# hbell99/DirectVoxGO

Measured on AMD Instinct MI355X. Metric: train rays/sec (8192-ray batch, 160^3 grid), higher is better.
Workload: dtype f32

## Files before the change

directvoxgo_amd/csrc/shade.hip:

```cpp
#include "common.h"
#include "x3.h"

#include <type_traits>


static int g_shade_experiment = 0;
static int g_shade_variant = 67;
extern "C" int dvgo_shade_wgrad_x3(const float* G1, const float* gz, const uint64_t* masks, const float* W3, const float* H1,
                                   const float* H2, const float* feat, int C, const float* emb, int E, const int64_t* ray_id,
                                   int64_t M, const int64_t* m_dev, int width, int diffuse, int n_parts, float* part, int form_b,
                                   void* stream);
extern "C" int dvgo_shade_bwd_x3(const float* g_rgb, const float* rgb, const uint64_t* masks, int64_t M, const int64_t* m_dev,
                                 const float* W1, const float* W2, const float* W3, int width, int d_in, int C, int diffuse,
                                 float* g_feat, float* G1, float* gz, void* scratch, int prebuilt, void* stream);

extern "C" int dvgo_shade_fwd_x3(const float* feat, int C, const float* emb, int E, const int64_t* ray_id, int64_t M, const int64_t* m_dev,
                                 const float* W1, const float* b1, const float* W2, const float* b2, const float* W3,
                                 const float* b3, int width, int d_in, int diffuse, float* rgb, float* H1, float* H2,
                                 uint64_t* masks, void* scratch, void* scratch_bwd, int experiment, void* stream);

#define SHADE_THREADS 768
#define SHADE_WAVES (SHADE_THREADS / 64)
#define SHADE_BWD_THREADS 1024
#define SHADE_BWD_WAVES (SHADE_BWD_THREADS / 64)
// ... 724 lines not shown
    if (j < 8) pb[2 * WIDTH + 8 * w + j] = (w == 0 && j < 3) ? sgz[j] : 0.0f;
    if (T == 2 && j >= 16) pb[2 * WIDTH + 16 * w + j] = 0.0f;
  }
#endif
}
typedef float dvgo_f32x2 __attribute__((ext_vector_type(2)));
template <int O0, int O1> __device__ __forceinline__ dvgo_f32x2 lds_f32_pair_st64(unsigned a) {
  dvgo_f32x2 v; asm volatile("ds_read2st64_b32 %0, %1 offset0:%2 offset1:%3" : "=v"(v) : "v"(a), "n"(O0), "n"(O1)); return v;
}
template <int O0, int O1> __device__ __forceinline__ dvgo_f32x2 lds_f32_pair(unsigned a) {
  dvgo_f32x2 v; asm volatile("ds_read2_b32 %0, %1 offset0:%2 offset1:%3" : "=v"(v) : "v"(a), "n"(O0), "n"(O1)); return v;
}
template <int OFF> __device__ __forceinline__ u32x4 lds_u32x4(unsigned a) {
  u32x4 v; asm volatile("ds_read_b128 %0, %1 offset:%2" : "=v"(v) : "v"(a), "n"(OFF)); return v;
}
template <int OFF> __device__ __forceinline__ void lds_store_u32x4(unsigned a, u32x4 v) {
  asm volatile("ds_write_b128 %0, %1 offset:%2" :: "v"(a), "v"(v), "n"(OFF) : "memory");
}

template <int WIDTH>
struct ShadeWgradRingX3 : ShadeWgradRing<WIDTH> {
  u32x4 fb[WIDTH / 32 + 2][3][64];
};

template <int WIDTH>
__global__ void __launch_bounds__(2 * WIDTH, 2)
shade_wgrad_ring_x3_kernel(const float* __restrict__ G1, const float* __restrict__ gz, const unsigned int* __restrict__ masks,
                           const float* __restrict__ W3, const float* __restrict__ H1, const float* __restrict__ H2,
                           const float* __restrict__ feat, int C, int c_view0, int n_view, const float* __restrict__ emb, int E,
                           const int64_t* __restrict__ ray_id, int64_t M_cap, const int64_t* __restrict__ m_dev,
// ... 231 lines not shown
#pragma unroll
  for (int c = 0; c < 3; ++c) {
    const float v = vW3[c] + __shfl_xor(vW3[c], 32);
    if (h == 0) pW3[c * WIDTH + 32 * w + j] = v;
    sgz[c] += __shfl_xor(sgz[c], 32);
  }
  sb1 += __shfl_xor(sb1, 32); sb2 += __shfl_xor(sb2, 32);
  if (h == 0) {
    pb[32 * w + j] = sb1;
    pb[WIDTH + 32 * w + j] = sb2;
    if (j < 8) pb[2 * WIDTH + 8 * w + j] = (w == 0 && j < 3) ? sgz[j] : 0.0f;
    if (T == 2 && j >= 16) pb[2 * WIDTH + 16 * w + j] = 0.0f;
  }
#endif
}
#undef DVGO_OOB

#define SHADE_REDUCE_SLICES 16
__global__ void __launch_bounds__(256)
shade_wgrad_reduce_kernel(const float* __restrict__ part, int n_parts, int n, int W, int d_in, float* __restrict__ out) {
  const int i = blockIdx.x * blockDim.x + threadIdx.x;
  if (i >= n) return;
  int o;
  const int nW2 = W * W, nW1 = W * 64, nW3 = 32 * W;
  if (i < nW2) o = i;
  else if (i < nW2 + nW1) {
    const int r = (i - nW2) >> 6, c = (i - nW2) & 63;
    o = c < d_in ? nW2 + r * d_in + c : -1;
  } else if (i < nW2 + nW1 + nW3) {
    const int e = i - nW2 - nW1;
// ... 18 lines not shown
    a3 += part[(int64_t)(p + 3) * n + i];
  }
  for (; p < p1; ++p) a0 += part[(int64_t)p * n + i];
  if (p1 > p0) atomicAdd(out + o, (a0 + a1) + (a2 + a3));
}

extern "C" {

int dvgo_shade_fwd(const float* feat, int C, const float* emb, int E, const int64_t* ray_id, int64_t M, const int64_t* m_dev,
                   const float* W1, const float* b1, const float* W2, const float* b2, const float* W3,
                   const float* b3, int width, int d_in, int diffuse, float* rgb, float* H1, float* H2,
                   uint64_t* masks, void* scratch, void* scratch_bwd, void* stream) {
  if (M < 0 || C <= 0 || E < 0) return DVGO_EINVAL;
  if (M == 0) return 0;
  if (!feat || !emb || !ray_id || !W1 || !b1 || !W2 || !b2 || !W3 || !b3 || !rgb) return DVGO_EINVAL;
  if ((H1 == nullptr) != (H2 == nullptr) || (H1 == nullptr) != (masks == nullptr)) return DVGO_EINVAL;
  const int c_view0 = diffuse ? 3 : 0;
  const int n_view = C - c_view0;
  if (n_view < 0 || d_in != n_view + E) return DVGO_EINVAL;
  if ((width != 128 && width != 64) || d_in > 40) return DVGO_ERANGE;
  if ((g_shade_variant & 1) && scratch != nullptr)
    return dvgo_shade_fwd_x3(feat, C, emb, E, ray_id, M, m_dev, W1, b1, W2, b2, W3, b3, width, d_in, diffuse, rgb, H1, H2, masks,
                             scratch, (g_shade_variant & 2) ? scratch_bwd : nullptr, g_shade_experiment, stream);
  hipStream_t s = (hipStream_t)stream;
  const int64_t n_tiles = (M + 31) / 32;
  const int64_t cap = width == 128 ? 256 : 512;
  int blocks = (int)((n_tiles + SHADE_WAVES - 1) / SHADE_WAVES < cap ? (n_tiles + SHADE_WAVES - 1) / SHADE_WAVES : cap);
#define DVGO_SHADE(W, S1, DIFF)                                                                           \
  shade_fwd_kernel<W, S1, DIFF><<<blocks, SHADE_THREADS, 0, s>>>(feat, C, c_view0, n_view, emb, E, ray_id, M, m_dev, W1, b1, W2, \
                                                          b2, W3, b3, d_in, rgb, H1, H2, (unsigned long long*)masks, g_shade_experiment)
  if (width == 128) {
    if (d_in <= 36) { if (diffuse) DVGO_SHADE(128, 18, true); else DVGO_SHADE(128, 18, false); }
    else            { if (diffuse) DVGO_SHADE(128, 20, true); else DVGO_SHADE(128, 20, false); }
  } else {
    if (d_in <= 12) { if (diffuse) DVGO_SHADE(64, 6, true); else DVGO_SHADE(64, 6, false); }
    else            { if (diffuse) DVGO_SHADE(64, 20, true); else DVGO_SHADE(64, 20, false); }
// ... 20 lines not shown
    return dvgo_shade_bwd_x3(g_rgb, rgb, masks, M, m_dev, W1, W2, W3, width, d_in, C, diffuse, g_feat, G1, gz, scratch, prebuilt, stream);
  hipStream_t s = (hipStream_t)stream;
  const int64_t n_tiles = (M + 31) / 32;
  const int64_t cap = width == 128 ? 256 : 512;
  int blocks = (int)((n_tiles + SHADE_BWD_WAVES - 1) / SHADE_BWD_WAVES < cap ? (n_tiles + SHADE_BWD_WAVES - 1) / SHADE_BWD_WAVES : cap);
#define DVGO_SHADE_BWD(W, DIFF)                                                                                                       \
  shade_bwd_kernel<W, DIFF><<<blocks, SHADE_BWD_THREADS, 0, s>>>(g_rgb, rgb, (const unsigned long long*)masks, M, m_dev, W1, W2, W3, d_in, C, c_view0, \
                                                            n_view, g_feat, G1, gz, g_shade_experiment)
  if (width == 128) { if (diffuse) DVGO_SHADE_BWD(128, true); else DVGO_SHADE_BWD(128, false); }
  else              { if (diffuse) DVGO_SHADE_BWD(64, true); else DVGO_SHADE_BWD(64, false); }
#undef DVGO_SHADE_BWD
  DVGO_LAUNCH_CHECK();
  return 0;
}

int dvgo_shade_wgrad(const float* G1, const float* gz, const uint64_t* masks, const float* W3, const float* H1,
                     const float* H2, const float* feat, int C, const float* emb, int E, const int64_t* ray_id, int64_t M,
                     const int64_t* m_dev, int width, int diffuse, int n_parts, float* part, float* total, void* stream) {
  if (M < 0 || n_parts <= 0 || C <= 0 || E < 0) return DVGO_EINVAL;
  if (!G1 || !gz || !masks || !W3 || !H1 || !H2 || !feat || !emb || !ray_id || !part || !total) return DVGO_EINVAL;
  const int c_view0 = diffuse ? 3 : 0;
  const int n_view = C - c_view0;
  if ((width != 128 && width != 64) || n_view < 0 || n_view + E > 40) return DVGO_ERANGE;
  bool ring = false;
  if (g_shade_variant & (4 | 32)) {
    const int form_b = (g_shade_variant & 32) ? 2 : (g_shade_variant & 16) ? 1 : 0;
    if (!form_b && n_parts > 256) n_parts = 256;
    const int rc = dvgo_shade_wgrad_x3(G1, gz, masks, W3, H1, H2, feat, C, emb, E, ray_id, M, m_dev, width, diffuse, n_parts, part,
                                       form_b, stream);
    if (rc != 0) return rc;
  } else if (!(g_shade_variant & 8) && n_view <= 16 && E <= 32 && (n_view + E <= 32 || (n_view % 4 == 0 && n_view >= 8)) &&
             M * width * 4 < ((int64_t)1 << 31) && M * C * 4 < ((int64_t)1 << 31)) {
    if (n_parts > 512) n_parts = 512;
    ring = true;
// ... 32 lines not shown
```

directvoxgo_amd/csrc/shade_x3.hip:

```cpp
#include "common.h"
#include "x3.h"

#ifndef X3_THREADS
#define X3_THREADS 512
#endif
#define X3_WAVES (X3_THREADS / 64)
#ifndef X3_BWD_THREADS
#define X3_BWD_THREADS 512
#endif
#define X3_BWD_WAVES (X3_BWD_THREADS / 64)
#define X3_STAGE_ROWS 16
#define X3_STAGE_STRIDE 36

__device__ __forceinline__ int x3_acc_feature(int t, int r, int h) { return 32 * t + (r & 3) + 8 * (r >> 2) + 4 * h; }

__device__ __forceinline__ void x3_split1(float v, unsigned short& s0, unsigned short& s1, unsigned short& s2) {
  const unsigned int h = x3_pack(v, 0.f) & 0xffffu;
  const float r = v - __uint_as_float(h << 16);
  const unsigned int m = x3_pack(r, 0.f) & 0xffffu;
  const float q = r - __uint_as_float(m << 16);
  s0 = (unsigned short)h; s1 = (unsigned short)m; s2 = (unsigned short)(x3_pack(q, 0.f) & 0xffffu);
}

template <int WIDTH, int KS1>
// ... 83 lines not shown
}

template <int WIDTH, int KS1, bool DIFFUSE>
__global__ void __launch_bounds__(X3_THREADS)
shade_fwd_x3_kernel(const float* __restrict__ feat, int C, int c_view0, int n_view, const float* __restrict__ emb, int E,
                    const int64_t* __restrict__ ray_id, int64_t M_cap, const int64_t* __restrict__ m_dev,
                    const void* __restrict__ image, float* __restrict__ rgb,
                    float* __restrict__ H1, float* __restrict__ H2, unsigned long long* __restrict__ masks, int experiment) {
  const int64_t M = m_dev ? (*m_dev < M_cap ? *m_dev : M_cap) : M_cap;
  constexpr int T = WIDTH / 32;
  __shared__ __attribute__((aligned(16))) X3Lds<WIDTH, KS1> L;
  x3_copy_image<X3Img<WIDTH, KS1>>(&L, image);
  __syncthreads();
  const int lane = threadIdx.x & 63, h = lane >> 5;
  float* stage = L.stage[threadIdx.x >> 6];
  const bool train = H1 != nullptr;
  const int64_t n_tiles = (M + 31) / 32;
  const int64_t gw = (int64_t)blockIdx.x * (blockDim.x >> 6) + (threadIdx.x >> 6);
  const int64_t nw = (int64_t)gridDim.x * (blockDim.x >> 6);
  const int d_in = n_view + E;
  const int64_t last = M > 0 ? M - 1 : 0;
  auto row_of = [&](int64_t tile) { const int64_t r = tile * 32 + (lane & 31); return r < M ? r : last; };
  float xin[KS1][8];
  auto load_inputs = [&](int64_t tile, int64_t rid) {
    const float* fr = feat + row_of(tile) * C + c_view0;
    const float* er = emb + rid * E - n_view;
#pragma unroll
    for (int s = 0; s < KS1; ++s)
#pragma unroll
      for (int j = 0; j < 8; ++j) {
        const int k = 16 * s + 8 * h + j;
// ... 22 lines not shown
#pragma unroll
    for (int t = 0; t < T; ++t) {
      f32x16 acc;
#pragma unroll
      for (int r = 0; r < 16; ++r) acc[r] = L.b1p[h][t * 16 + r];
#pragma unroll
      for (int s = 0; s < KS1; ++s)
        x3_mfma6(acc, L.w1s[t][s][0][lane], L.w1s[t][s][1][lane], L.w1s[t][s][2][lane], x3[s][0], x3[s][1], x3[s][2]);
#pragma unroll
      for (int r = 0; r < 16; ++r) acc[r] = dvgo_relu(acc[r]);
      if (train) {
        unsigned int bits = 0u;
#pragma unroll
        for (int r = 0; r < 16; ++r) bits |= dvgo_relu_bit(acc[r]) << r;
        mask1 |= (unsigned long long)bits << (16 * t);
        if (!(experiment & 512)) x3_store_tile(stage, acc, H1 + tile * 32 * WIDTH + 32 * t, WIDTH, lane, rows_valid);
      }
#pragma unroll
      for (int s2 = 0; s2 < 2; ++s2) {
        float v[8];
#pragma unroll
        for (int j = 0; j < 8; ++j) v[j] = acc[8 * s2 + j];
        x3_split8(v, h3[2 * t + s2][0], h3[2 * t + s2][1], h3[2 * t + s2][2]);
      }
      __builtin_amdgcn_sched_barrier(0);
    }
    float p[3] = {0.0f, 0.0f, 0.0f};
    unsigned long long mask2 = 0ull;
#pragma unroll 1
    for (int t2 = 0; t2 < T; ++t2) {
      f32x16 acc2;
// ... 908 lines not shown
extern "C" {

int64_t dvgo_shade_scratch_bytes(int width) {
  if (width == 128) return (int64_t)sizeof(X3Img<128, 3>) > (int64_t)sizeof(X3BwdImg<128>) ? sizeof(X3Img<128, 3>) : sizeof(X3BwdImg<128>);
  if (width == 64) return (int64_t)sizeof(X3Img<64, 3>) > (int64_t)sizeof(X3BwdImg<64>) ? sizeof(X3Img<64, 3>) : sizeof(X3BwdImg<64>);
  return 0;
}

int dvgo_shade_fwd_x3(const float* feat, int C, const float* emb, int E, const int64_t* ray_id, int64_t M, const int64_t* m_dev,
                      const float* W1, const float* b1, const float* W2, const float* b2, const float* W3,
                      const float* b3, int width, int d_in, int diffuse, float* rgb, float* H1, float* H2,
                      uint64_t* masks, void* scratch, void* scratch_bwd, int experiment, void* stream) {
  if (M < 0 || C <= 0 || E < 0) return DVGO_EINVAL;
  if (M == 0) return 0;
  if (!feat || !emb || !ray_id || !W1 || !b1 || !W2 || !b2 || !W3 || !b3 || !rgb || !scratch) return DVGO_EINVAL;
  if ((H1 == nullptr) != (H2 == nullptr) || (H1 == nullptr) != (masks == nullptr)) return DVGO_EINVAL;
  const int c_view0 = diffuse ? 3 : 0;
  const int n_view = C - c_view0;
  if (n_view < 0 || d_in != n_view + E) return DVGO_EINVAL;
  if ((width != 128 && width != 64) || d_in > 48) return DVGO_ERANGE;
  hipStream_t s = (hipStream_t)stream;
  const int64_t n_tiles = (M + 31) / 32;
  const int64_t cap = 256;
  const int blocks = (int)((n_tiles + X3_WAVES - 1) / X3_WAVES < cap ? (n_tiles + X3_WAVES - 1) / X3_WAVES : cap);
#define DVGO_SHADE_X3(W, KS, DIFF)                                                                                       \
  do {                                                                                                                   \
    x3_prep_fwd_kernel<W, KS><<<scratch_bwd ? 64 : 32, 256, 0, s>>>((X3Img<W, KS>*)scratch, (X3BwdImg<W>*)scratch_bwd, W1, b1, W2, b2, W3, b3, d_in); \
    shade_fwd_x3_kernel<W, KS, DIFF><<<blocks, X3_THREADS, 0, s>>>(feat, C, c_view0, n_view, emb, E, ray_id, M, m_dev, scratch, rgb, \
                                                                    H1, H2, (unsigned long long*)masks, experiment);     \
  } while (0)
  if (width == 128) {
// ... 71 lines not shown
```

directvoxgo_amd/shade.py:

```python

import torch
import torch.nn as nn

from . import _lib as L
from ._lib import _i64, _int, ptr, stream_of

N_PARTS = 512


class defer_wgrad:
    _active = None
    _streams = {}

    def __init__(self, side_stream=True):
        self.side_stream = side_stream

    def __enter__(self):
        self.pending = []
        defer_wgrad._active = self
        return self

    def __exit__(self, *exc):
        defer_wgrad._active = None
        return False
# ... 64 lines not shown
        defer_wgrad._active.submit(params, wgrad, device)
    else:
        grads[k:k + 6] = wgrad()
    return tuple(grads)


class _Shade(torch.autograd.Function):
    @staticmethod
    def forward(ctx, feat, emb, ray_id, W1, b1, W2, b2, W3, b3, diffuse, train, m_dev):
        M, C = feat.shape
        E = emb.shape[1]
        width, d_in = W1.shape
        feat, emb = feat.contiguous(), emb.contiguous()
        train = bool(train) and any(ctx.needs_input_grad)
        rgb = torch.empty((M, 3), dtype=torch.float32, device=feat.device)
        H1 = torch.empty((M, width), dtype=torch.float32, device=feat.device) if train else None
        H2 = torch.empty((M, width), dtype=torch.float32, device=feat.device) if train else None
        masks = torch.empty((M, 4), dtype=torch.int64, device=feat.device) if train else None
        scratch = _scratch(width, feat.device)
        scratch_bwd = _scratch(width, feat.device) if (train and (L.lib().dvgo_shade_variant(-1) & 2)) else None
        with L.device_of(feat):
            L.call('dvgo_shade_fwd', ptr(feat), _int(C), ptr(emb), _int(E), ptr(ray_id), _i64(M), ptr(m_dev), ptr(W1.contiguous()),
                   ptr(b1.contiguous()), ptr(W2.contiguous()), ptr(b2.contiguous()), ptr(W3.contiguous()),
                   ptr(b3.contiguous()), _int(width), _int(d_in), _int(1 if diffuse else 0), ptr(rgb), ptr(H1), ptr(H2),
                   ptr(masks), ptr(scratch), ptr(scratch_bwd), stream_of(feat))
        ctx.scratch_bwd = scratch_bwd if (train and (L.lib().dvgo_shade_variant(-1) & 1)) else None
        if train:
            ctx.save_for_backward(feat, emb, ray_id, W1, W2, W3, rgb, H1, H2, masks)
            ctx.diffuse = diffuse
            ctx.m_dev = m_dev
            ctx.params = (W1, b1, W2, b2, W3, b3)
            ctx.w_versions = (W1._version, W2._version, W3._version)
        return rgb

    @staticmethod
    @torch.autograd.function.once_differentiable
    def backward(ctx, g_rgb):
        feat, emb, ray_id, W1, W2, W3, rgb, H1, H2, masks = ctx.saved_tensors
        diffuse, m_dev = ctx.diffuse, ctx.m_dev
        M, C = feat.shape
        width, d_in = W1.shape
        g_feat = torch.empty_like(feat)
        G1 = torch.empty_like(H1)
        gz = torch.empty_like(rgb)
        prebuilt = ctx.scratch_bwd is not None and W1._version == ctx.w_versions[0] and W2._version == ctx.w_versions[1] \
            and W3._version == ctx.w_versions[2]
        scratch = ctx.scratch_bwd if prebuilt else _scratch(width, feat.device)
        ctx.scratch_bwd = None
        with L.device_of(feat):
            L.call('dvgo_shade_bwd', ptr(g_rgb.contiguous()), ptr(rgb), ptr(masks), _i64(M), ptr(m_dev), ptr(W1.contiguous()),
                   ptr(W2.contiguous()), ptr(W3.contiguous()), _int(width), _int(d_in), _int(C), _int(1 if diffuse else 0),
                   ptr(g_feat), ptr(G1), ptr(gz), ptr(scratch), _int(1 if prebuilt else 0), stream_of(feat))

        def wgrad():
            n_parts = max(1, min(N_PARTS, (M + 255) // 256))
            psize = width * width + width * 64 + 32 * width + 3 * width
            part = torch.empty((n_parts, psize), dtype=torch.float32, device=feat.device)
            tsize = width * width + width * d_in + 5 * width + 3
            tot = torch.empty(tsize, dtype=torch.float32, device=feat.device)
            with L.device_of(feat):
                L.call('dvgo_shade_wgrad', ptr(G1), ptr(gz), ptr(masks), ptr(W3.contiguous()), ptr(H1), ptr(H2), ptr(feat), _int(C), ptr(emb),
                       _int(emb.shape[1]), ptr(ray_id), _i64(M), ptr(m_dev), _int(width), _int(1 if diffuse else 0), _int(n_parts),
                       ptr(part), ptr(tot), stream_of(feat))
            return _unpack_record(tot, width, d_in)

        return _weight_grads(ctx.params, wgrad, feat.device, 3, 12, g_feat if ctx.needs_input_grad[0] else None)


def shade(rgbnet, feat, emb, ray_id, diffuse, m_dev=None):
    layers = head_layers(rgbnet)
    if layers is None or not feat.is_cuda:
        return None
    l1, l2, l3 = layers
    c0 = 3 if diffuse else 0
    if l1.in_features != feat.shape[1] - c0 + emb.shape[1]:
# ... 92 lines not shown
```

include/dvgo_hip.h:

```cpp
#ifndef DVGO_HIP_H
#define DVGO_HIP_H

#include <stdint.h>

#ifdef __cplusplus
extern "C" {
#endif

#define DVGO_EINVAL (-1)
#define DVGO_ERANGE (-2)

#define DVGO_ABI_VERSION 11
int dvgo_abi_version(void);

#define DVGO_TUNE_FEAT_BWD    0
#define DVGO_TUNE_DENSITY_BWD 1
#define DVGO_TUNE_DENSITY_FWD 2
#define DVGO_TUNE_GATHER      3
#define DVGO_TUNE_EXPERIMENT  4
#define DVGO_TUNE_COUNT       8
int dvgo_set_tuning(int key, int value);

int dvgo_infer_t_minmax(const float* rays_o, const float* rays_d,
                        const float* xyz_min, const float* xyz_max,
// ... 176 lines not shown
                   void* stream);

int64_t dvgo_shade_scratch_bytes(int width);
int dvgo_shade_variant(int flags);

int dvgo_shade_bwd(const float* g_rgb, const float* rgb, const uint64_t* masks, int64_t M, const int64_t* m_dev,
                   const float* W1, const float* W2, const float* W3, int width, int d_in, int C, int diffuse,
                   float* g_feat, float* G1, float* gz, void* scratch,
                   int prebuilt ,
                   void* stream);

int dvgo_shade_wgrad(const float* G1, const float* gz, const uint64_t* masks, const float* W3,
                     const float* H1, const float* H2, const float* feat, int C, const float* emb, int E, const int64_t* ray_id, int64_t M,
                     const int64_t* m_dev, int width, int diffuse, int n_parts, float* part, float* total, void* stream);

int dvgo_march_positions(const float* rays_start, const float* rays_dir, const int64_t* ray_id, const int64_t* step_id,
                         int64_t M, float stepdist, float* pts, void* stream);
int dvgo_shade_pe_fwd(const float* pts, const float* freq, int P, const float* emb, int E, const int64_t* ray_id, int64_t M,
                      const float* W1, const float* b1, const float* W2, const float* b2, const float* W3, const float* b3,
                      int width, int d_in, float* rgb, float* H1, float* H2, uint64_t* masks, void* stream);
int dvgo_shade_pe_bwd(const float* g_rgb, const float* rgb, const uint64_t* masks, int64_t M, const float* W2,
                      const float* W3, int width, float* G1, float* gz, void* stream);
int64_t dvgo_shade_pe_record_size(int width, int d_in);
int dvgo_shade_pe_wgrad(const float* G1, const float* gz, const uint64_t* masks, const float* W3, const float* H1,
                        const float* H2, const float* pts, const float* freq, int P, const float* emb, int E,
                        const int64_t* ray_id, int64_t M, int width, int d_in, int n_parts, float* part, float* total,
                        void* stream);

int dvgo_adam_upd(float* param, const float* grad, float* exp_avg, float* exp_avg_sq,
                  const float* perlr , int64_t n, float step_size,
// ... 195 lines not shown
```

Measured before the change: 3.093 million.

## Recompute layer-1 activations in weight-grad kernel instead of storing H1

Adds a weight-gradient kernel that recomputes the first-layer activations (H1) on the fly from features, embeddings, W1 and b1 using split-bf16 MFMA, so the forward pass no longer writes H1 and the backward pass no longer reads it. This removes an M×width fp32 store and load per training step in exchange for extra matrix-core work and more LDS staging in the wgrad kernel. W1/b1 are passed through a thread-local side channel, and the variant flag is changed so the new path is enabled by default.

```diff
diff --git a/directvoxgo_amd/csrc/shade.hip b/directvoxgo_amd/csrc/shade.hip
--- a/directvoxgo_amd/csrc/shade.hip
+++ b/directvoxgo_amd/csrc/shade.hip
@@ -5,7 +5,7 @@
 
 
 static int g_shade_experiment = 0;
-static int g_shade_variant = 67;
+static int g_shade_variant = 195;
 extern "C" int dvgo_shade_wgrad_x3(const float* G1, const float* gz, const uint64_t* masks, const float* W3, const float* H1,
                                    const float* H2, const float* feat, int C, const float* emb, int E, const int64_t* ray_id,
                                    int64_t M, const int64_t* m_dev, int width, int diffuse, int n_parts, float* part, int form_b,
@@ -762,6 +762,10 @@
 template <int OFF> __device__ __forceinline__ u32x4 lds_u32x4(unsigned a) {
   u32x4 v; asm volatile("ds_read_b128 %0, %1 offset:%2" : "=v"(v) : "v"(a), "n"(OFF)); return v;
 }
+typedef float dvgo_f32x3 __attribute__((ext_vector_type(3)));
+template <int OFF> __device__ __forceinline__ dvgo_f32x3 lds_f32x3(unsigned a) {
+  dvgo_f32x3 v; asm volatile("ds_read_b96 %0, %1 offset:%2" : "=v"(v) : "v"(a), "n"(OFF)); return v;
+}
 template <int OFF> __device__ __forceinline__ void lds_store_u32x4(unsigned a, u32x4 v) {
   asm volatile("ds_write_b128 %0, %1 offset:%2" :: "v"(a), "v"(v), "n"(OFF) : "memory");
 }
@@ -1023,6 +1027,357 @@
   }
 #endif
 }
+template <int WIDTH>
+struct ShadeWgradRingH1 {
+  static constexpr int NB = 2, NS = 3, NR = 4, TR = 16;
+  float g1[NB][TR][WIDTH], h2[NB][TR][WIDTH];
+  float xf[NS][TR][16];
+  float xe[NS][TR][32];
+  float gz[NB][TR][4];
+  unsigned int m2[NB][TR][4];
+  unsigned int rid[NR][64];
+  u32x4 fh[2][WIDTH / 32][3][64];
+  u32x4 fx[2][3][64];
+};
+
+template <int WIDTH>
+__global__ void __launch_bounds__(2 * WIDTH, 2)
+shade_wgrad_ring_h1_kernel(const float* __restrict__ G1, const float* __restrict__ gz, const unsigned int* __restrict__ masks,
+                           const float* __restrict__ W3, const float* __restrict__ W1, const float* __restrict__ b1,
+                           const float* __restrict__ H2, const float* __restrict__ feat, int C, int c_view0, int n_view,
+                           const float* __restrict__ emb, int E, const int64_t* __restrict__ ray_id, int64_t M_cap,
+                           const int64_t* __restrict__ m_dev, float* __restrict__ part, float* __restrict__ total, int total_size) {
+#if defined(__HIP_DEVICE_COMPILE__)
+  for (int i = blockIdx.x * blockDim.x + threadIdx.x; i < total_size; i += gridDim.x * blockDim.x) total[i] = 0.0f;
+  int64_t M;
+  {
+    const int64_t m = m_dev ? (*m_dev < M_cap ? *m_dev : M_cap) : M_cap;
+    M = ((int64_t)__builtin_amdgcn_readfirstlane((int)(m >> 32)) << 32) | (unsigned)__builtin_amdgcn_readfirstlane((int)m);
+  }
+  using Ring = ShadeWgradRingH1<WIDTH>;
+  constexpr int T = WIDTH / 32, NW = T, NB = Ring::NB, NR = Ring::NR, TR = Ring::TR;
+  static_assert(T == 4 || T == 2, "widths 128 and 64");
+  static_assert(sizeof(Ring) <= 81920, "two workgroups per CU");
+  constexpr int LPR = WIDTH / 4, RPI = 64 / LPR, IPW = TR / RPI / NW;
+  constexpr int DW = NW == 4 ? 2 : NW, FPW = 4 / DW, EPW = 8 / DW;
+  static_assert(IPW == 2 && NB == 2 && TR == 16 && EPW == 4, "double buffer of 16-row tiles: the wait at the top of a tile is vmcnt(0)");
+  __shared__ __attribute__((aligned(16))) Ring L;
+  const int tid = threadIdx.x, lane = tid & 63, h = lane >> 5, j = lane & 31;
+  const int w = __builtin_amdgcn_readfirstlane(tid >> 6);
+  const int dw = NW == 4 ? w - 2 : w;
+  f32x16 aW2[T], aW1[2];
+  float vW3[3] = {0.0f, 0.0f, 0.0f}, sgz[3] = {0.0f, 0.0f, 0.0f};
+#pragma unroll
+  for (int t = 0; t < T; ++t)
+#pragma unroll
+    for (int r = 0; r < 16; ++r) aW2[t][r] = 0.0f;
+#pragma unroll
+  for (int q = 0; q < 2; ++q)
+#pragma unroll
+    for (int r = 0; r < 16; ++r) aW1[q][r] = 0.0f;
+  float sb1 = 0.0f, sb2 = 0.0f;
+  const float w30 = W3[32 * w + j], w31 = W3[WIDTH + 32 * w + j], w32 = W3[2 * WIDTH + 32 * w + j];
+  const int m_idx = 2 * ((j >> 2) & 1) + (w >> 1);
+  const unsigned m_bit = 16 * (w & 1) + (j & 3) + 4 * (j >> 3);
+  const int d_in = n_view + E;
+  u32x4 w1f[3][3];
+#pragma unroll
+  for (int s = 0; s < 3; ++s) {
+    float v[8];
+#pragma unroll
+    for (int e = 0; e < 8; ++e) {
+      const int c = 16 * s + 8 * h + e;
+      v[e] = c < d_in ? W1[(32 * w + j) * d_in + c] : 0.0f;
+    }
+    x3_split8(v, w1f[s][0], w1f[s][1], w1f[s][2]);
+  }
+  const float b1v = b1[32 * w + j];
+  const int n_tiles = (int)((M + TR - 1) / TR);
+  auto tile_of = [&](int k) { return (int)blockIdx.x + k * (int)gridDim.x; };
+  const unsigned rows_b = (unsigned)(M * WIDTH * 4);
+  const auto bG1 = __builtin_amdgcn_make_buffer_rsrc((void*)G1, 0, rows_b, 0x00020000);
+  const auto bH2 = __builtin_amdgcn_make_buffer_rsrc((void*)H2, 0, rows_b, 0x00020000);
+  const auto bF = __builtin_amdgcn_make_buffer_rsrc((void*)feat, 0, (unsigned)(M * C * 4), 0x00020000);
+  const auto bE = __builtin_amdgcn_make_buffer_rsrc((void*)emb, 0, DVGO_OOB, 0x00020000);
+  const auto bGz = __builtin_amdgcn_make_buffer_rsrc((void*)gz, 0, (unsigned)(M * 12), 0x00020000);
+  const auto bM = __builtin_amdgcn_make_buffer_rsrc((void*)masks, 0, (unsigned)(M * 32), 0x00020000);
+  const auto bR = __builtin_amdgcn_make_buffer_rsrc((void*)ray_id, 0, (unsigned)(M * 8), 0x00020000);
+  unsigned vo_bulk[IPW], vo_f[FPW], vo_ecol[EPW];
+#pragma unroll
+  for (int i = 0; i < IPW; ++i) vo_bulk[i] = (unsigned)(((IPW * w + i) * RPI + lane / LPR) * WIDTH * 4 + 16 * (lane % LPR));
+#pragma unroll
+  for (int i = 0; i < FPW; ++i) {
+    const int e = 64 * ((dw < 0 ? 0 : dw) + DW * i) + lane, row = e >> 4, col = e & 15;
+    vo_f[i] = col < n_view ? (unsigned)((row * C + c_view0 + col) * 4) : DVGO_OOB;
+  }
+#pragma unroll
+  for (int i = 0; i < EPW; ++i) {
+    const int e = 64 * ((dw < 0 ? 0 : dw) + DW * i) + lane, col = e & 31;
+    vo_ecol[i] = col < E ? (unsigned)(col * 4) : DVGO_OOB;
+  }
+  const unsigned vo_gz = (lane & 3) < 3 ? (unsigned)(((lane >> 2) * 3 + (lane & 3)) * 4) : DVGO_OOB;
+  const unsigned vo_m2 = (unsigned)(((lane >> 2) * 8 + 4 + (lane & 3)) * 4);
+  const unsigned vo_rid = (unsigned)((lane & (TR - 1)) * 8);
+  const unsigned a_rid = lds_addr(&L.rid[0][2 * (dw < 0 ? 0 : dw) + h]);
+  auto issue_bulk = [&](int t) {
+    const int sl = t & (NB - 1);
+    const unsigned r0 = (unsigned)__builtin_amdgcn_readfirstlane(tile_of(t) * TR);
+#pragma unroll
+    for (int i = 0; i < IPW; ++i) {
+      const int rl = (IPW * w + i) * RPI;
+      __builtin_amdgcn_raw_ptr_buffer_load_lds(bG1, (dvgo_lptr_t)&L.g1[sl][rl][0], 16, vo_bulk[i], r0 * (WIDTH * 4), 0, 0);
+      __builtin_amdgcn_raw_ptr_buffer_load_lds(bH2, (dvgo_lptr_t)&L.h2[sl][rl][0], 16, vo_bulk[i], r0 * (WIDTH * 4), 0, 0);
+    }
+    if (dw == 0) {
+      __builtin_amdgcn_raw_ptr_buffer_load_lds(bGz, (dvgo_lptr_t)&L.gz[sl][0][0], 4, vo_gz, r0 * 12u, 0, 0);
+      __builtin_amdgcn_raw_ptr_buffer_load_lds(bM, (dvgo_lptr_t)&L.m2[sl][0][0], 4, vo_m2, r0 * 32u, 0, 0);
+    }
+  };
+  auto issue_x = [&](int t, int sl3 ) {
+    if (dw < 0) return;
+    const unsigned r0 = (unsigned)__builtin_amdgcn_readfirstlane(tile_of(t) * TR);
+#pragma unroll
+    for (int i = 0; i < FPW; ++i)
+      __builtin_amdgcn_raw_ptr_buffer_load_lds(bF, (dvgo_lptr_t)(&L.xf[sl3][0][0] + 64 * (dw + DW * i)), 4, vo_f[i], r0 * (unsigned)(C * 4), 0, 0);
+    unsigned rids[EPW];
+    asm volatile("ds_read_b32 %0, %4\n\tds_read_b32 %1, %4 offset:%5\n\tds_read_b32 %2, %4 offset:%6\n\tds_read_b32 %3, %4 offset:%7\n\t"
+                 "s_waitcnt lgkmcnt(0)"
+                 : "=&v"(rids[0]), "=&v"(rids[1]), "=&v"(rids[2]), "=&v"(rids[3])
+                 : "v"(a_rid + (unsigned)((t & (NR - 1)) * 256)), "n"(8 * DW), "n"(16 * DW), "n"(24 * DW));
+#pragma unroll
+    for (int i = 0; i < EPW; ++i)
+      __builtin_amdgcn_raw_ptr_buffer_load_lds(bE, (dvgo_lptr_t)(&L.xe[sl3][0][0] + 64 * (dw + DW * i)), 4,
+                                               vo_ecol[i] + rids[i] * (unsigned)(E * 4), 0, 0, 0);
+  };
+  auto issue_rid = [&](int t) {
+    if (dw != 1) return;
+    const unsigned rn = (unsigned)__builtin_amdgcn_readfirstlane(tile_of(t) * TR);
+    __builtin_amdgcn_raw_ptr_buffer_load_lds(bR, (dvgo_lptr_t)&L.rid[t & (NR - 1)][0], 4, vo_rid, rn * 8u, 0, 0);
+  };
+#define DVGO_H1_ROW(e) (((e) & 3) + 8 * ((e) >> 2))
+  const unsigned a_gz = lds_addr(&L.gz[0][4 * h][0]), a_mw = lds_addr(&L.m2[0][4 * h][m_idx]);
+  const unsigned a_g1 = lds_addr(&L.g1[0][4 * h][32 * w + j]);
+  static_assert(offsetof(Ring, h2) - offsetof(Ring, g1) == sizeof(L.g1) && offsetof(Ring, fx) - offsetof(Ring, fh) == sizeof(L.fh), "");
+  constexpr int H2_OFF = (int)sizeof(L.g1) / 256;
+  constexpr unsigned FX_OFF = (unsigned)sizeof(L.fh);
+  const int xcol = 32 * (w & 1) + j;
+  const bool x_in_f = xcol < n_view, x_ok = xcol < d_in;
+  const unsigned a_x = x_in_f ? lds_addr(&L.xf[0][4 * h][xcol]) : lds_addr(&L.xe[0][4 * h][x_ok ? xcol - n_view : 0]);
+  const unsigned a_rf = lds_addr(&L.xf[0][j & 15][8 * h]);
+  const unsigned a_re = lds_addr(&L.xe[0][j & 15][8 * h]) - (unsigned)(4 * n_view);
+  const int nv_h = n_view - 8 * h, din_h = d_in - 8 * h;
+  const unsigned a_fh = lds_addr(&L.fh[0][0][0][lane]);
+  constexpr unsigned SLOT_ROWS = TR * WIDTH * 4, FB_TILE = 3 * 64 * 16, FB_PIECE = 64 * 16;
+  constexpr unsigned XF_SLOT = TR * 16 * 4, XE_SLOT = TR * 32 * 4;
+  if (tid < 64) {
+#pragma unroll
+    for (int t = 0; t < 3; ++t) {
+      const int64_t row = (int64_t)tile_of(t) * TR + (tid & (TR - 1));
+      L.rid[t][tid] = row < M ? (unsigned int)ray_id[row] : 0u;
+    }
+  }
+  __syncthreads();
+  issue_x(0, 0);
+  issue_x(1, 1);
+  issue_bulk(0);
+  int k3 = 0;
+  for (int k = 0; tile_of(k) < n_tiles; ++k) {
+    const int sl = k & (NB - 1);
+    const int k3n = k3 == 2 ? 0 : k3 + 1, k3nn = k3n == 2 ? 0 : k3n + 1;
+    asm volatile("s_waitcnt vmcnt(0)\n\ts_waitcnt lgkmcnt(0)\n\ts_barrier" ::: "memory");
+    issue_bulk(k + 1);
+    issue_x(k + 2, k3nn);
+    issue_rid(k + 3);
+    if (!(k & 1)) {
+      const int xs = j < 16 ? k3 : k3n;
+      const unsigned b_rf = a_rf + xs * XF_SLOT, b_re = a_re + xs * XE_SLOT;
+      float xr[3][8];
+      {
+        unsigned ad[8];
+#pragma unroll
+        for (int e = 0; e < 8; ++e) ad[e] = e < nv_h ? b_rf : b_re;
+        asm volatile("ds_read_b32 %0, %8\n\tds_read_b32 %1, %9 offset:4\n\tds_read_b32 %2, %10 offset:8\n\tds_read_b32 %3, %11 offset:12\n\t"
+                     "ds_read_b32 %4, %12 offset:16\n\tds_read_b32 %5, %13 offset:20\n\tds_read_b32 %6, %14 offset:24\n\t"
+                     "ds_read_b32 %7, %15 offset:28\n\ts_waitcnt lgkmcnt(0)"
+                     : "=&v"(xr[0][0]), "=&v"(xr[0][1]), "=&v"(xr[0][2]), "=&v"(xr[0][3]), "=&v"(xr[0][4]), "=&v"(xr[0][5]), "=&v"(xr[0][6]),
+                       "=&v"(xr[0][7])
+                     : "v"(ad[0]), "v"(ad[1]), "v"(ad[2]), "v"(ad[3]), "v"(ad[4]), "v"(ad[5]), "v"(ad[6]), "v"(ad[7]));
+        asm volatile("ds_read_b32 %0, %16 offset:64\n\tds_read_b32 %1, %16 offset:68\n\tds_read_b32 %2, %16 offset:72\n\t"
+                     "ds_read_b32 %3, %16 offset:76\n\tds_read_b32 %4, %16 offset:80\n\tds_read_b32 %5, %16 offset:84\n\t"
+                     "ds_read_b32 %6, %16 offset:88\n\tds_read_b32 %7, %16 offset:92\n\t"
+                     "ds_read_b32 %8, %16 offset:128\n\tds_read_b32 %9, %16 offset:132\n\tds_read_b32 %10, %16 offset:136\n\t"
+                     "ds_read_b32 %11, %16 offset:140\n\tds_read_b32 %12, %16 offset:144\n\tds_read_b32 %13, %16 offset:148\n\t"
+                     "ds_read_b32 %14, %16 offset:152\n\tds_read_b32 %15, %16 offset:156\n\ts_waitcnt lgkmcnt(0)"
+                     : "=&v"(xr[1][0]), "=&v"(xr[1][1]), "=&v"(xr[1][2]), "=&v"(xr[1][3]), "=&v"(xr[1][4]), "=&v"(xr[1][5]), "=&v"(xr[1][6]),
+                       "=&v"(xr[1][7]), "=&v"(xr[2][0]), "=&v"(xr[2][1]), "=&v"(xr[2][2]), "=&v"(xr[2][3]), "=&v"(xr[2][4]), "=&v"(xr[2][5]),
+                       "=&v"(xr[2][6]), "=&v"(xr[2][7])
+                     : "v"(b_re));
+      }
+#pragma unroll
+      for (int e = 0; e < 8; ++e) xr[2][e] = (32 + e) < din_h ? xr[2][e] : 0.0f;
+      f32x16 acc;
+#pragma unroll
+      for (int r = 0; r < 16; ++r) acc[r] = b1v;
+#define X3D_MF(ACC, A, B) ACC = __builtin_amdgcn_mfma_f32_32x32x16_bf16(__builtin_bit_cast(bf16x8, A), __builtin_bit_cast(bf16x8, B), ACC, 0, 0, 0)
+#pragma unroll
+      for (int s = 0; s < 3; ++s) {
+        u32x4 x0, x1, x2;
+        x3_split8(xr[s], x0, x1, x2);
+        X3D_MF(acc, x0, w1f[s][2]); X3D_MF(acc, x1, w1f[s][1]); X3D_MF(acc, x2, w1f[s][0]);
+        X3D_MF(acc, x0, w1f[s][1]); X3D_MF(acc, x1, w1f[s][0]);
+        X3D_MF(acc, x0, w1f[s][0]);
+        __builtin_amdgcn_sched_barrier(0);
+      }
+#undef X3D_MF
+#pragma unroll
+      for (int s2 = 0; s2 < 2; ++s2) {
+        float v[8];
+#pragma unroll
+        for (int e = 0; e < 8; ++e) v[e] = dvgo_relu(acc[8 * s2 + e]);
+        u32x4 p0, p1, p2;
+        x3_split8(v, p0, p1, p2);
+        lds_store_u32x4<0>(a_fh + (s2 * T + w) * FB_TILE, p0);
+        lds_store_u32x4<FB_PIECE>(a_fh + (s2 * T + w) * FB_TILE, p1);
+        lds_store_u32x4<2 * FB_PIECE>(a_fh + (s2 * T + w) * FB_TILE, p2);
+        __builtin_amdgcn_sched_barrier(0);
+      }
+    }
+    const unsigned b_gz = a_gz + sl * (TR * 16), b_mw = a_mw + sl * (TR * 16), b_g1 = a_g1 + sl * SLOT_ROWS;
+    const unsigned b_x = a_x + k3 * (x_in_f ? XF_SLOT : XE_SLOT);
+    dvgo_f32x3 gq[8];
+    dvgo_f32x2 mwp[4];
+    unsigned mw[8];
+    float g1v[8], h2v[8], xv[8];
+    constexpr int RS = WIDTH * 4 / 256;
+    if (w < 2) {
+#define DVGO_H1_XV(ST)                                                                                                            \
+  asm volatile("ds_read_b32 %0, %8\n\tds_read_b32 %1, %8 offset:%9\n\tds_read_b32 %2, %8 offset:%10\n\tds_read_b32 %3, %8 offset:%11\n\t" \
+               "ds_read_b32 %4, %8 offset:%12\n\tds_read_b32 %5, %8 offset:%13\n\tds_read_b32 %6, %8 offset:%14\n\t"           \
+               "ds_read_b32 %7, %8 offset:%15\n\ts_waitcnt lgkmcnt(0)"                                                          \
+               : "=&v"(xv[0]), "=&v"(xv[1]), "=&v"(xv[2]), "=&v"(xv[3]), "=&v"(xv[4]), "=&v"(xv[5]), "=&v"(xv[6]), "=&v"(xv[7])   \
+               : "v"(b_x), "n"(1 * (ST)), "n"(2 * (ST)), "n"(3 * (ST)), "n"(8 * (ST)), "n"(9 * (ST)), "n"(10 * (ST)), "n"(11 * (ST)))
+      if (x_in_f) DVGO_H1_XV(16 * 4); else DVGO_H1_XV(32 * 4);
+#undef DVGO_H1_XV
+    }
+    asm volatile("ds_read_b96 %0, %12\n\tds_read_b96 %1, %12 offset:16\n\tds_read_b96 %2, %12 offset:32\n\tds_read_b96 %3, %12 offset:48\n\t"
+                 "ds_read_b96 %4, %12 offset:128\n\tds_read_b96 %5, %12 offset:144\n\tds_read_b96 %6, %12 offset:160\n\t"
+                 "ds_read_b96 %7, %12 offset:176\n\t"
+                 "ds_read2_b32 %8, %13 offset0:0 offset1:4\n\tds_read2_b32 %9, %13 offset0:8 offset1:12\n\t"
+                 "ds_read2_b32 %10, %13 offset0:32 offset1:36\n\tds_read2_b32 %11, %13 offset0:40 offset1:44\n\t"
+                 "s_waitcnt lgkmcnt(0)"
+                 : "=&v"(gq[0]), "=&v"(gq[1]), "=&v"(gq[2]), "=&v"(gq[3]), "=&v"(gq[4]), "=&v"(gq[5]), "=&v"(gq[6]), "=&v"(gq[7]),
+                   "=&v"(mwp[0]), "=&v"(mwp[1]), "=&v"(mwp[2]), "=&v"(mwp[3])
+                 : "v"(b_gz), "v"(b_mw));
+#pragma unroll
+    for (int e = 0; e < 4; ++e) { mw[2 * e] = __float_as_uint(mwp[e].x); mw[2 * e + 1] = __float_as_uint(mwp[e].y); }
+    if (w < 2) {
+#pragma unroll
+      for (int e = 0; e < 8; ++e) xv[e] = x_ok ? xv[e] : 0.0f;
+      u32x4 p0, p1, p2;
+      x3_split8(xv, p0, p1, p2);
+      lds_store_u32x4<FX_OFF>(a_fh + w * FB_TILE, p0);
+      lds_store_u32x4<FX_OFF + FB_PIECE>(a_fh + w * FB_TILE, p1);
+      lds_store_u32x4<FX_OFF + 2 * FB_PIECE>(a_fh + w * FB_TILE, p2);
+    }
+    __builtin_amdgcn_sched_barrier(0);
+    u32x4 a2f[3], a1f[3];
+    {
+      float a2[8];
+#pragma unroll
+      for (int e = 0; e < 8; ++e) {
+        const float g2v = fmaf(w32, gq[e].z, fmaf(w31, gq[e].y, w30 * gq[e].x));
+        a2[e] = __uint_as_float(__float_as_uint(g2v) & (unsigned)__builtin_amdgcn_sbfe((int)mw[e], m_bit, 1u));
+        sb2 += a2[e];
+      }
+      if (w == 0) {
+#pragma unroll
+        for (int e = 0; e < 8; ++e) { sgz[0] += gq[e].x; sgz[1] += gq[e].y; sgz[2] += gq[e].z; }
+      }
+      x3_split8(a2, a2f[0], a2f[1], a2f[2]);
+      {
+        dvgo_f32x2 ga, gb, gc, gd, ha, hb, hc, hd;
+        asm volatile("ds_read2st64_b32 %0, %8 offset0:%9 offset1:%10\n\tds_read2st64_b32 %1, %8 offset0:%11 offset1:%12\n\t"
+                     "ds_read2st64_b32 %2, %8 offset0:%13 offset1:%14\n\tds_read2st64_b32 %3, %8 offset0:%15 offset1:%16\n\t"
+                     "ds_read2st64_b32 %4, %8 offset0:%17 offset1:%18\n\tds_read2st64_b32 %5, %8 offset0:%19 offset1:%20\n\t"
+                     "ds_read2st64_b32 %6, %8 offset0:%21 offset1:%22\n\tds_read2st64_b32 %7, %8 offset0:%23 offset1:%24\n\t"
+                     "s_waitcnt lgkmcnt(0)"
+                     : "=&v"(ga), "=&v"(gb), "=&v"(gc), "=&v"(gd), "=&v"(ha), "=&v"(hb), "=&v"(hc), "=&v"(hd)
+                     : "v"(b_g1), "n"(0 * RS), "n"(1 * RS), "n"(2 * RS), "n"(3 * RS), "n"(8 * RS), "n"(9 * RS), "n"(10 * RS), "n"(11 * RS),
+                       "n"(H2_OFF + 0 * RS), "n"(H2_OFF + 1 * RS), "n"(H2_OFF + 2 * RS), "n"(H2_OFF + 3 * RS), "n"(H2_OFF + 8 * RS),
+                       "n"(H2_OFF + 9 * RS), "n"(H2_OFF + 10 * RS), "n"(H2_OFF + 11 * RS));
+        g1v[0] = ga.x; g1v[1] = ga.y; g1v[2] = gb.x; g1v[3] = gb.y; g1v[4] = gc.x; g1v[5] = gc.y; g1v[6] = gd.x; g1v[7] = gd.y;
+        h2v[0] = ha.x; h2v[1] = ha.y; h2v[2] = hb.x; h2v[3] = hb.y; h2v[4] = hc.x; h2v[5] = hc.y; h2v[6] = hd.x; h2v[7] = hd.y;
+      }
+#pragma unroll
+      for (int e = 0; e < 8; ++e) {
+        sb1 += g1v[e];
+        vW3[0] = fmaf(gq[e].x, h2v[e], vW3[0]); vW3[1] = fmaf(gq[e].y, h2v[e], vW3[1]); vW3[2] = fmaf(gq[e].z, h2v[e], vW3[2]);
+      }
+      x3_split8(g1v, a1f[0], a1f[1], a1f[2]);
+    }
+    asm volatile("s_waitcnt lgkmcnt(0)\n\ts_barrier" ::: "memory");
+    u32x4 fr[2][3];
+    auto read_pair = [&](unsigned base, auto Oc, u32x4 (&f)[2][3]) {
+      constexpr unsigned o = decltype(Oc)::value;
+      asm volatile("ds_read_b128 %0, %6 offset:%7\n\tds_read_b128 %1, %6 offset:%8\n\tds_read_b128 %2, %6 offset:%9\n\t"
+                   "ds_read_b128 %3, %6 offset:%10\n\tds_read_b128 %4, %6 offset:%11\n\tds_read_b128 %5, %6 offset:%12\n\t"
+                   "s_waitcnt lgkmcnt(0)"
+                   : "=&v"(f[0][0]), "=&v"(f[0][1]), "=&v"(f[0][2]), "=&v"(f[1][0]), "=&v"(f[1][1]), "=&v"(f[1][2])
+                   : "v"(base), "n"(o), "n"(o + FB_PIECE), "n"(o + 2 * FB_PIECE), "n"(o + FB_TILE), "n"(o + FB_TILE + FB_PIECE),
+                     "n"(o + FB_TILE + 2 * FB_PIECE));
+    };
+    auto mfma_pair = [&](f32x16& accA, f32x16& accB, const u32x4 (&a)[3], const u32x4 (&f)[2][3]) {
+#define X3D_MF(ACC, A, B) ACC = __builtin_amdgcn_mfma_f32_32x32x16_bf16(__builtin_bit_cast(bf16x8, A), __builtin_bit_cast(bf16x8, B), ACC, 0, 0, 0)
+      X3D_MF(accA, a[2], f[0][0]); X3D_MF(accB, a[2], f[1][0]);
+      X3D_MF(accA, a[1], f[0][1]); X3D_MF(accB, a[1], f[1][1]);
+      X3D_MF(accA, a[0], f[0][2]); X3D_MF(accB, a[0], f[1][2]);
+      X3D_MF(accA, a[1], f[0][0]); X3D_MF(accB, a[1], f[1][0]);
+      X3D_MF(accA, a[0], f[0][1]); X3D_MF(accB, a[0], f[1][1]);
+      X3D_MF(accA, a[0], f[0][0]); X3D_MF(accB, a[0], f[1][0]);
+#undef X3D_MF
+    };
+    constexpr int NP = T / 2 + 1;
+    const unsigned b_fh = a_fh + (k & 1) * (T * FB_TILE);
+    static_for<0, NP>([&](auto Pc) {
+      constexpr int p = decltype(Pc)::value;
+      if constexpr (p < T / 2) read_pair(b_fh, std::integral_constant<unsigned, 2 * p * FB_TILE>{}, fr);
+      else read_pair(a_fh, std::integral_constant<unsigned, FX_OFF>{}, fr);
+      if constexpr (p < T / 2) mfma_pair(aW2[2 * p], aW2[2 * p + 1], a2f, fr);
+      else mfma_pair(aW1[0], aW1[1], a1f, fr);
+      __builtin_amdgcn_sched_barrier(0);
+    });
+    k3 = k3n;
+  }
+#undef DVGO_H1_ROW
+  asm volatile("s_waitcnt vmcnt(0)" ::: "memory");
+  float* p = part + (int64_t)blockIdx.x * (WIDTH * WIDTH + WIDTH * 64 + 32 * WIDTH + 3 * WIDTH);
+  float* pW2 = p;
+  float* pW1 = pW2 + WIDTH * WIDTH;
+  float* pW3 = pW1 + WIDTH * 64;
+  float* pb = pW3 + 32 * WIDTH;
+#pragma unroll
+  for (int r = 0; r < 16; ++r) {
+    const int i = (r & 3) + 8 * (r >> 2) + 4 * h;
+#pragma unroll
+    for (int t = 0; t < T; ++t) pW2[(32 * w + i) * WIDTH + 32 * t + j] = aW2[t][r];
+    pW1[(32 * w + i) * 64 + j] = aW1[0][r];
+    pW1[(32 * w + i) * 64 + 32 + j] = aW1[1][r];
+  }
+#pragma unroll
+  for (int c = 0; c < 3; ++c) {
+    const float v = vW3[c] + __shfl_xor(vW3[c], 32);
+    if (h == 0) pW3[c * WIDTH + 32 * w + j] = v;
+    sgz[c] += __shfl_xor(sgz[c], 32);
+  }
+  sb1 += __shfl_xor(sb1, 32); sb2 += __shfl_xor(sb2, 32);
+  if (h == 0) {
+    pb[32 * w + j] = sb1;
+    pb[WIDTH + 32 * w + j] = sb2;
+    if (j < 8) pb[2 * WIDTH + 8 * w + j] = (w == 0 && j < 3) ? sgz[j] : 0.0f;
+    if (T == 2 && j >= 16) pb[2 * WIDTH + 16 * w + j] = 0.0f;
+  }
+#endif
+}
 #undef DVGO_OOB
 
 #define SHADE_REDUCE_SLICES 16
@@ -1071,12 +1426,14 @@
   if (M < 0 || C <= 0 || E < 0) return DVGO_EINVAL;
   if (M == 0) return 0;
   if (!feat || !emb || !ray_id || !W1 || !b1 || !W2 || !b2 || !W3 || !b3 || !rgb) return DVGO_EINVAL;
-  if ((H1 == nullptr) != (H2 == nullptr) || (H1 == nullptr) != (masks == nullptr)) return DVGO_EINVAL;
+  const bool x3 = (g_shade_variant & 1) && scratch != nullptr;
+  if ((H2 == nullptr) != (masks == nullptr) || (H1 != nullptr && H2 == nullptr)) return DVGO_EINVAL;
+  if (H1 == nullptr && H2 != nullptr && !x3) return DVGO_EINVAL;
   const int c_view0 = diffuse ? 3 : 0;
   const int n_view = C - c_view0;
   if (n_view < 0 || d_in != n_view + E) return DVGO_EINVAL;
   if ((width != 128 && width != 64) || d_in > 40) return DVGO_ERANGE;
-  if ((g_shade_variant & 1) && scratch != nullptr)
+  if (x3)
     return dvgo_shade_fwd_x3(feat, C, emb, E, ray_id, M, m_dev, W1, b1, W2, b2, W3, b3, width, d_in, diffuse, rgb, H1, H2, masks,
                              scratch, (g_shade_variant & 2) ? scratch_bwd : nullptr, g_shade_experiment, stream);
   hipStream_t s = (hipStream_t)stream;
@@ -1127,10 +1484,62 @@
   return 0;
 }
 
+int dvgo_shade_wgrad_reads_h1(int width, int C, int E, int diffuse, int64_t M) {
+  const int n_view = C - (diffuse ? 3 : 0);
+  const bool rebuild = (g_shade_variant & (128 | 64 | 1)) == (128 | 64 | 1) && !(g_shade_variant & (4 | 8 | 32)) &&
+                       (width == 128 || width == 64) && n_view >= 0 && n_view <= 16 && E >= 0 && E <= 32 && n_view + E <= 40 &&
+                       M >= 0 && M * width * 4 < ((int64_t)1 << 31) && M * C * 4 < ((int64_t)1 << 31);
+  return rebuild ? 0 : 1;
+}
+
+static thread_local const float* g_wgrad_W1 = nullptr;
+static thread_local const float* g_wgrad_b1 = nullptr;
+int dvgo_shade_wgrad_layer1(const float* W1, const float* b1) {
+  if (!W1 || !b1) return DVGO_EINVAL;
+  g_wgrad_W1 = W1; g_wgrad_b1 = b1;
+  return 0;
+}
+
+static int shade_wgrad_h1(const float* G1, const float* gz, const uint64_t* masks, const float* W3, const float* W1, const float* b1,
+                          const float* H2, const float* feat, int C, const float* emb, int E, const int64_t* ray_id, int64_t M,
+                          const int64_t* m_dev, int width, int diffuse, int n_parts, float* part, float* total, void* stream) {
+  if (M < 0 || n_parts <= 0 || C <= 0 || E < 0) return DVGO_EINVAL;
+  if (M == 0 && total && (width == 128 || width == 64) && C - (diffuse ? 3 : 0) >= 0)
+    return hipMemsetAsync(total, 0, (size_t)(width * width + width * (C - (diffuse ? 3 : 0) + E) + 5 * width + 3) * sizeof(float),
+                          (hipStream_t)stream) == hipSuccess ? 0 : DVGO_EINVAL;
+  if (!G1 || !gz || !masks || !W3 || !W1 || !b1 || !H2 || !feat || !emb || !ray_id || !part || !total) return DVGO_EINVAL;
+  if (dvgo_shade_wgrad_reads_h1(width, C, E, diffuse, M)) return DVGO_ERANGE;
+  const int c_view0 = diffuse ? 3 : 0;
+  const int n_view = C - c_view0, d_in = n_view + E;
+  if (n_parts > 512) n_parts = 512;
+  const int tsz = width * width + width * d_in + 5 * width + 3;
+  if (width == 128)
+    shade_wgrad_ring_h1_kernel<128><<<n_parts, 256, 0, (hipStream_t)stream>>>(
+        G1, gz, (const unsigned int*)masks, W3, W1, b1, H2, feat, C, c_view0, n_view, emb, E, ray_id, M, m_dev, part, total, tsz);
+  else
+    shade_wgrad_ring_h1_kernel<64><<<n_parts, 128, 0, (hipStream_t)stream>>>(
+        G1, gz, (const unsigned int*)masks, W3, W1, b1, H2, feat, C, c_view0, n_view, emb, E, ray_id, M, m_dev, part, total, tsz);
+  DVGO_LAUNCH_CHECK();
+  const int psize = width * width + width * 64 + 32 * width + 3 * width;
+  shade_wgrad_reduce_kernel<<<dim3((psize + 255) / 256, SHADE_REDUCE_SLICES), 256, 0, (hipStream_t)stream>>>(part, n_parts, psize,
+                                                                                                       width, d_in, total);
+  DVGO_LAUNCH_CHECK();
+  return 0;
+}
+
 int dvgo_shade_wgrad(const float* G1, const float* gz, const uint64_t* masks, const float* W3, const float* H1,
                      const float* H2, const float* feat, int C, const float* emb, int E, const int64_t* ray_id, int64_t M,
                      const int64_t* m_dev, int width, int diffuse, int n_parts, float* part, float* total, void* stream) {
   if (M < 0 || n_parts <= 0 || C <= 0 || E < 0) return DVGO_EINVAL;
+  if (M == 0 && total && (width == 128 || width == 64) && C - (diffuse ? 3 : 0) >= 0)
+    return hipMemsetAsync(total, 0, (size_t)(width * width + width * (C - (diffuse ? 3 : 0) + E) + 5 * width + 3) * sizeof(float),
+                          (hipStream_t)stream) == hipSuccess ? 0 : DVGO_EINVAL;
+  if (H1 == nullptr) {
+    const float* W1 = g_wgrad_W1;
+    const float* b1 = g_wgrad_b1;
+    g_wgrad_W1 = g_wgrad_b1 = nullptr;
+    return shade_wgrad_h1(G1, gz, masks, W3, W1, b1, H2, feat, C, emb, E, ray_id, M, m_dev, width, diffuse, n_parts, part, total, stream);
+  }
   if (!G1 || !gz || !masks || !W3 || !H1 || !H2 || !feat || !emb || !ray_id || !part || !total) return DVGO_EINVAL;
   const int c_view0 = diffuse ? 3 : 0;
   const int n_view = C - c_view0;
diff --git a/directvoxgo_amd/csrc/shade_x3.hip b/directvoxgo_amd/csrc/shade_x3.hip
--- a/directvoxgo_amd/csrc/shade_x3.hip
+++ b/directvoxgo_amd/csrc/shade_x3.hip
@@ -121,7 +121,7 @@
   __syncthreads();
   const int lane = threadIdx.x & 63, h = lane >> 5;
   float* stage = L.stage[threadIdx.x >> 6];
-  const bool train = H1 != nullptr;
+  const bool train = masks != nullptr;
   const int64_t n_tiles = (M + 31) / 32;
   const int64_t gw = (int64_t)blockIdx.x * (blockDim.x >> 6) + (threadIdx.x >> 6);
   const int64_t nw = (int64_t)gridDim.x * (blockDim.x >> 6);
@@ -174,7 +174,7 @@
 #pragma unroll
         for (int r = 0; r < 16; ++r) bits |= dvgo_relu_bit(acc[r]) << r;
         mask1 |= (unsigned long long)bits << (16 * t);
-        if (!(experiment & 512)) x3_store_tile(stage, acc, H1 + tile * 32 * WIDTH + 32 * t, WIDTH, lane, rows_valid);
+        if (H1 != nullptr && !(experiment & 512)) x3_store_tile(stage, acc, H1 + tile * 32 * WIDTH + 32 * t, WIDTH, lane, rows_valid);
       }
 #pragma unroll
       for (int s2 = 0; s2 < 2; ++s2) {
@@ -1113,7 +1113,7 @@
   if (M < 0 || C <= 0 || E < 0) return DVGO_EINVAL;
   if (M == 0) return 0;
   if (!feat || !emb || !ray_id || !W1 || !b1 || !W2 || !b2 || !W3 || !b3 || !rgb || !scratch) return DVGO_EINVAL;
-  if ((H1 == nullptr) != (H2 == nullptr) || (H1 == nullptr) != (masks == nullptr)) return DVGO_EINVAL;
+  if ((H2 == nullptr) != (masks == nullptr) || (H1 != nullptr && H2 == nullptr)) return DVGO_EINVAL;
   const int c_view0 = diffuse ? 3 : 0;
   const int n_view = C - c_view0;
   if (n_view < 0 || d_in != n_view + E) return DVGO_EINVAL;
diff --git a/directvoxgo_amd/shade.py b/directvoxgo_amd/shade.py
--- a/directvoxgo_amd/shade.py
+++ b/directvoxgo_amd/shade.py
@@ -102,7 +102,8 @@
         feat, emb = feat.contiguous(), emb.contiguous()
         train = bool(train) and any(ctx.needs_input_grad)
         rgb = torch.empty((M, 3), dtype=torch.float32, device=feat.device)
-        H1 = torch.empty((M, width), dtype=torch.float32, device=feat.device) if train else None
+        keep_h1 = train and bool(L.lib().dvgo_shade_wgrad_reads_h1(width, C, E, 1 if diffuse else 0, M))
+        H1 = torch.empty((M, width), dtype=torch.float32, device=feat.device) if keep_h1 else None
         H2 = torch.empty((M, width), dtype=torch.float32, device=feat.device) if train else None
         masks = torch.empty((M, 4), dtype=torch.int64, device=feat.device) if train else None
         scratch = _scratch(width, feat.device)
@@ -114,7 +115,7 @@
                    ptr(masks), ptr(scratch), ptr(scratch_bwd), stream_of(feat))
         ctx.scratch_bwd = scratch_bwd if (train and (L.lib().dvgo_shade_variant(-1) & 1)) else None
         if train:
-            ctx.save_for_backward(feat, emb, ray_id, W1, W2, W3, rgb, H1, H2, masks)
+            ctx.save_for_backward(feat, emb, ray_id, W1, W2, W3, rgb, H1, H2, masks, b1)
             ctx.diffuse = diffuse
             ctx.m_dev = m_dev
             ctx.params = (W1, b1, W2, b2, W3, b3)
@@ -124,12 +125,12 @@
     @staticmethod
     @torch.autograd.function.once_differentiable
     def backward(ctx, g_rgb):
-        feat, emb, ray_id, W1, W2, W3, rgb, H1, H2, masks = ctx.saved_tensors
+        feat, emb, ray_id, W1, W2, W3, rgb, H1, H2, masks, b1 = ctx.saved_tensors
         diffuse, m_dev = ctx.diffuse, ctx.m_dev
         M, C = feat.shape
         width, d_in = W1.shape
         g_feat = torch.empty_like(feat)
-        G1 = torch.empty_like(H1)
+        G1 = torch.empty_like(H2)
         gz = torch.empty_like(rgb)
         prebuilt = ctx.scratch_bwd is not None and W1._version == ctx.w_versions[0] and W2._version == ctx.w_versions[1] \
             and W3._version == ctx.w_versions[2]
@@ -147,6 +148,8 @@
             tsize = width * width + width * d_in + 5 * width + 3
             tot = torch.empty(tsize, dtype=torch.float32, device=feat.device)
             with L.device_of(feat):
+                if H1 is None:
+                    L.call('dvgo_shade_wgrad_layer1', ptr(W1.contiguous()), ptr(b1.contiguous()))
                 L.call('dvgo_shade_wgrad', ptr(G1), ptr(gz), ptr(masks), ptr(W3.contiguous()), ptr(H1), ptr(H2), ptr(feat), _int(C), ptr(emb),
                        _int(emb.shape[1]), ptr(ray_id), _i64(M), ptr(m_dev), _int(width), _int(1 if diffuse else 0), _int(n_parts),
                        ptr(part), ptr(tot), stream_of(feat))
diff --git a/include/dvgo_hip.h b/include/dvgo_hip.h
--- a/include/dvgo_hip.h
+++ b/include/dvgo_hip.h
@@ -214,6 +214,9 @@
                      const float* H1, const float* H2, const float* feat, int C, const float* emb, int E, const int64_t* ray_id, int64_t M,
                      const int64_t* m_dev, int width, int diffuse, int n_parts, float* part, float* total, void* stream);
 
+int dvgo_shade_wgrad_reads_h1(int width, int C, int E, int diffuse, int64_t M);
+int dvgo_shade_wgrad_layer1(const float* W1, const float* b1);
+
 int dvgo_march_positions(const float* rays_start, const float* rays_dir, const int64_t* ray_id, const int64_t* step_id,
                          int64_t M, float stepdist, float* pts, void* stream);
 int dvgo_shade_pe_fwd(const float* pts, const float* freq, int P, const float* emb, int E, const int64_t* ray_id, int64_t M,
```

After: 2.830 million. 0.915x the previous value.
